# aicodix/modem

Measured on AMD Instinct MI355X. Metric: decoded frames/sec + BER, mode-6 8kHz OFDM, batch 65536, 1/2/4/8 MI355X, higher is better.
Workload: dtype f32

## Files before the change

modem_amd/csrc/dev_common.h:

```cpp
#pragma once
#include <hip/hip_runtime.h>
#include <stdint.h>

#if defined(BACK_WALK) || defined(DEMOD_QA_LDS) || defined(DEMOD_RAW_AHEAD) || defined(DEMOD_SWZ) || defined(DEMOD_TWR_BYTES) || defined(POLAR_NT_LEVEL) || defined(POLAR_WPB) || defined(POLAR_XB1) || defined(POLAR_XB2) || defined(POLAR_XB3) || defined(SYNC_FFT_IN_LDS) || defined(SYNC_PER) || defined(SYNC_SPLIT_8K) || defined(SYNC_SPLIT_ROUNDS) || defined(SYNC_WAVES) || defined(SYNC_WAVES_SPLIT_MONO) || defined(TS_CAP) || defined(TS_MARGIN) || defined(TS_MORE_OCC) || defined(TS_MORE_WAVES_N) || defined(TS_OPEN_MARGIN) || defined(TS_OPEN_NEED) || defined(TS_OWN_ATAN) || defined(TS_ROWS_PER_WG) || defined(TS_UNC_STEPS) || defined(TX_NT_LDS) || defined(TX_TW_GLOBAL)
#error "a frozen tuning macro was passed with -D: edit a patched copy of the source instead (tools/experiments/ts_stage_probe.py shows how)"
#endif

namespace rx {

template <int RATE> struct RateCfg {
	static constexpr int SL = (int)((1280L * RATE) / 8000);
	static constexpr int FILTER_LEN = (((21 * RATE) / 8000) & ~3) | 1;
	static constexpr int GL = SL / 8;
	static constexpr int STRIDE = SL + GL;
	static constexpr int HS = SL / 2;
	static constexpr int BUFFER_LEN = 6 * STRIDE;
	static constexpr int SEARCH_POS = BUFFER_LEN - 4 * STRIDE;
	static constexpr int MATCH_LEN = GL | 1;
	static constexpr int MATCH_DEL = (MATCH_LEN - 1) / 2;
};
inline bool rate_supported(int rate) { return rate == 8000 || rate == 16000 || rate == 44100 || rate == 48000; }
inline int rate_symbol_len(int rate) { return (int)((1280L * rate) / 8000); }
inline int rate_filter_len(int rate) { return (((21 * rate) / 8000) & ~3) | 1; }
#define RX_RATE_SWITCH(rate, ...) \
// ... 27 lines not shown
constexpr int MESG_BITS_MAX = 44096;
constexpr int MESG_BYTES_MAX = 5512;

struct ModeDesc { int cols, rows, mod_bits, cons_bits, mesg_bits, table; };
__host__ __device__ inline ModeDesc mode_desc(int mode)
{
	ModeDesc m;
	m.table = mode >= 10;
	m.cons_bits = m.table ? 64512 : 64800;
	m.mesg_bits = m.table ? 44096 : 43808;
	switch (mode) {
	case 6: m.cols = 432; m.mod_bits = 3; break;
	case 7: m.cols = 400; m.mod_bits = 3; break;
	case 8: m.cols = 400; m.mod_bits = 2; break;
	case 9: m.cols = 360; m.mod_bits = 2; break;
	case 10: m.cols = 512; m.mod_bits = 3; break;
	case 11: m.cols = 384; m.mod_bits = 3; break;
	case 12: m.cols = 384; m.mod_bits = 2; break;
	default: m.cols = 256; m.mod_bits = 2; break;
	}
	m.rows = (m.cons_bits / m.mod_bits) / m.cols;
	return m;
}

struct cf { float re, im; };

__device__ __forceinline__ cf mk(float re, float im) { cf r; r.re = re; r.im = im; return r; }
__device__ __forceinline__ cf cadd(cf a, cf b) { return mk(a.re + b.re, a.im + b.im); }
__device__ __forceinline__ cf csub(cf a, cf b) { return mk(a.re - b.re, a.im - b.im); }
__device__ __forceinline__ cf cmul(cf a, cf b) { return mk(a.re * b.re - a.im * b.im, a.re * b.im + a.im * b.re); }
__device__ __forceinline__ cf cconj(cf a) { return mk(a.re, -a.im); }
__device__ __forceinline__ float cnorm(cf a) { return a.re * a.re + a.im * a.im; }
__device__ __forceinline__ cf cmul_negj(cf a) { return mk(a.im, -a.re); }

__device__ __forceinline__ cf demod_or_erase(cf curr, cf prev)
{
	float d = cnorm(prev);
	if (!(d > 0.f))
		return mk(0.f, 0.f);
	cf n = cmul(curr, cconj(prev));
	cf c = mk(n.re / d, n.im / d);
	if (!(cnorm(c) <= 4.f))
		return mk(0.f, 0.f);
	return c;
}

__device__ __forceinline__ cf psk4_hard_map(cf c)
{
	const float r = 0.70710678118654752440f;
	return mk(r * (c.re < 0.f ? -1.f : 1.f), r * (c.im < 0.f ? -1.f : 1.f));
}
__device__ __forceinline__ cf psk8_hard_map(cf c)
{
	const float cos_pi_8 = 0.92387953251128675613f, sin_pi_8 = 0.38268343236508977173f;
	float b1 = c.re < 0.f ? -1.f : 1.f;
	float b2 = c.im < 0.f ? -1.f : 1.f;
	bool swap = fabsf(c.re) < fabsf(c.im);
	float real = swap ? sin_pi_8 : cos_pi_8, imag = swap ? cos_pi_8 : sin_pi_8;
	return mk(real * b1, imag * b2);
}

__device__ __forceinline__ cf phasor(float omega, long k)
{
	double a = (double)omega * (double)k;
	const double inv2pi = 0.15915494309189533577, twopi = 6.28318530717958647692;
	a -= twopi * rint(a * inv2pi);
	float s, c;
	sincosf((float)a, &s, &c);
	return mk(c, s);
}

__device__ __forceinline__ float div_32767(float x)
{
	const float c = 1.0f / 32767.f;
	const float q0 = x * c;
	return __builtin_fmaf(__builtin_fmaf(-32767.f, q0, x), c, q0);
}
__device__ __forceinline__ float div_127(float x)
{
	const float c = 1.0f / 127.f;
	const float q0 = x * c;
	return __builtin_fmaf(__builtin_fmaf(-127.f, q0, x), c, q0);
}

template <int FMT> __device__ __forceinline__ float2 iq_sample(const void *in, size_t i)
{
	if (FMT == 0) {
		const short2 v = ((const short2 *)in)[i];
		return make_float2(div_32767((float)v.x), div_32767((float)v.y));
	}
	if (FMT == 1) {
		const unsigned v = ((const uint16_t *)in)[i];
		return make_float2(div_127((float)((int)(v & 255u) - 128)), div_127((float)((int)(v >> 8) - 128)));
	}
	return ((const float2 *)in)[i];
}

__device__ __forceinline__ void phase_phasor(unsigned phase, float &cs, float &sn)
{
	const float x = (float)(int)phase * (1.f / 4294967296.f);
	sincospif(2.f * x, &sn, &cs);
}

__device__ __forceinline__ long long floor_div(long long a, int d)
{
	const long long q = a / d;
	return q * d > a ? q - 1 : q;
}

template <int OFMT> __device__ __forceinline__ void iq_store(void *out, long long t0, int t, float wr, float wi)
{
	if (OFMT == 0) {
		const float re = fminf(fmaxf(wr + 0.f, -1.f), 1.f), im = fminf(fmaxf(wi + 0.f, -1.f), 1.f);
		((short2 *)out)[t0 + t] = make_short2((short)nearbyintf(32767.f * re), (short)nearbyintf(32767.f * im));
	} else {
		((float2 *)out)[t0 + t] = make_float2(wr + 0.f, wi + 0.f);
	}
}

template <int V> struct IntC { static constexpr int value = V; };
struct SampleSrc {
	const void *base;
	int fmt;
	int channels;
	long n;
	const cf *analytic;
	__device__ __forceinline__ cf at(long i) const
	{
		if (i < 0 || i >= n)
			return mk(0.f, 0.f);
		if (analytic)
			return analytic[i];
		if (fmt == 0) {
			short2 v = ((const short2 *)base)[i];
			return mk(div_32767((float)v.x), div_32767((float)v.y));
		}
		return pair_other(i);
	}
	__device__ __forceinline__ cf pair_other(long i) const
	{
		if (fmt == 1) {
			const unsigned v = ((const uint16_t *)base)[i];
			return mk(div_127((float)((int)(v & 255u) - 128)), div_127((float)((int)(v >> 8) - 128)));
		}
		const float2 v = ((const float2 *)base)[i];
		return mk(v.x, v.y);
	}
	__device__ __forceinline__ int mode() const { return analytic ? 0 : (fmt == 0 ? 1 : 2); }
	template <int M> __device__ __forceinline__ cf at_m(long i) const
	{
		if (i < 0 || i >= n)
			return mk(0.f, 0.f);
		if (M == 0)
			return analytic[i];
		if (M == 1) {
			short2 v = ((const short2 *)base)[i];
			return mk(div_32767((float)v.x), div_32767((float)v.y));
		}
		return pair_other(i);
	}
	template <class F> __device__ __forceinline__ void with_mode(F f) const
	{
		const int m = mode();
		if (m == 0) f(IntC<0>{});
		else if (m == 1) f(IntC<1>{});
		else f(IntC<2>{});
// ... 95 lines not shown
			Bfly<R>::run(v[q]);
		}
	}
	fft_sync<NT>();
	#pragma unroll
	for (int q = 0; q < NB; ++q) {
		int b = tid + q * NT;
		if (b < T) {
			int k = b % P;
			int j = (b - k) * R + k;
			#pragma unroll
			for (int t = 0; t < R; ++t)
				buf[j + t * P] = v[q][t];
		}
	}
	fft_sync<NT>();
}

template <int N, int REM, int P, int NT, int TWN, int TWC> struct FftPlan {
	static constexpr int R = REM % 5 == 0 ? 5 : REM % 7 == 0 ? 7 : REM % 3 == 0 ? 3 : REM % 4 == 0 ? 4 : 2;
	static constexpr int OWN = P > 1 ? (R - 1) * P : 0;
	using Next = FftPlan<N, REM / R, P * R, NT, TWN, (TWC >= 0 ? TWC + OWN : -1)>;
	static constexpr int COMPACT = OWN + Next::COMPACT;
	static __device__ __forceinline__ void run(cf *buf, const cf *tw, int tid)
	{
		fft_stage<N, R, P, NT, TWN, TWC>(buf, tw, tid);
		Next::run(buf, tw, tid);
	}
	static __device__ __forceinline__ void fill(cf *dst, const cf *src, int tid)
	{
		if (P > 1)
			for (int i = tid; i < OWN; i += NT)
				dst[TWC + i] = src[((i / P + 1) * (i % P)) * (TWN / (P * R))];
		Next::fill(dst, src, tid);
	}
};
template <int N, int P, int NT, int TWN, int TWC> struct FftPlan<N, 1, P, NT, TWN, TWC> {
	static constexpr int COMPACT = 0;
	static __device__ __forceinline__ void run(cf *, const cf *, int) {}
	static __device__ __forceinline__ void fill(cf *, const cf *, int) {}
};
template <int N, int NT, int TWN>
__device__ __forceinline__ void fft_fwd(cf *buf, const cf *tw, int tid)
{
	FftPlan<N, N, 1, NT, TWN, -1>::run(buf, tw, tid);
}
template <int N, int TWN> constexpr int fft_compact_size() { return FftPlan<N, N, 1, 64, TWN, 0>::COMPACT; }
template <int N, int NT, int TWN>
__device__ __forceinline__ void fft_compact_twiddles(cf *dst, const cf *tw, int tid)
{
	FftPlan<N, N, 1, NT, TWN, 0>::fill(dst, tw, tid);
}
template <int N, int NT, int TWN>
__device__ __forceinline__ void fft_fwd_compact(cf *buf, const cf *twc, int tid)
{
	FftPlan<N, N, 1, NT, TWN, 0>::run(buf, twc, tid);
}

__device__ __forceinline__ int swz256(int i) { return i ^ ((i >> 2) & 3) ^ (((i >> 4) & 3) << 2); }
template <int P, int TWC> __device__ __forceinline__ void fft256_stage_swz(cf *buf, const cf *tw, int lane, int sl)
{
	cf v[4];
	const int k = lane % P;
	#pragma unroll
	for (int t = 0; t < 4; ++t) {
		cf x = buf[sl + t * 64];
		if (t && P > 1)
			x = cmul(x, tw[TWC + (t - 1) * P + k]);
		v[t] = x;
	}
	Bfly<4>::run(v);
	fft_sync<64>();
	const int j = (lane - k) * 4 + k;
	#pragma unroll
	for (int t = 0; t < 4; ++t)
		buf[swz256(j + t * P)] = v[t];
	fft_sync<64>();
}

__host__ __device__ constexpr int fft256_pos(int q)
{
	return (q & 192) | ((q & 3) << 4) | (q & 12) | ((q >> 4) & 3);
}
template <int NT> __device__ __forceinline__ void fft256_lane_twiddles(cf *twl, const cf *tw1280, int tid)
{
	for (int i = tid; i < 9 * 64; i += NT) {
		const int l = i & 63, k = (i >> 6) % 3 + 1, step = i / 192;
		const int e = step == 0 ? 5 * (l * k) : step == 1 ? 20 * ((l & 15) * k) : 80 * ((l & 3) * k);
		twl[i] = tw1280[e % 1280];
	}
}
template <int BIT> __device__ __forceinline__ void fft256_xchg(float &A, float &B, int lane)
{
	const int a = __float_as_int(A), b = __float_as_int(B);
	if constexpr (BIT == 5) {
		auto r = __builtin_amdgcn_permlane32_swap((unsigned)a, (unsigned)b, false, false);
		A = __int_as_float((int)r[0]); B = __int_as_float((int)r[1]);
	} else if constexpr (BIT == 4) {
		auto r = __builtin_amdgcn_permlane16_swap((unsigned)a, (unsigned)b, false, false);
		A = __int_as_float((int)r[0]); B = __int_as_float((int)r[1]);
	} else if constexpr (BIT == 3) {
		A = __int_as_float(__builtin_amdgcn_update_dpp(a, b, 0x128, 0xf, 0xC, false));
		B = __int_as_float(__builtin_amdgcn_update_dpp(b, a, 0x128, 0xf, 0x3, false));
	} else if constexpr (BIT == 2) {
		A = __int_as_float(__builtin_amdgcn_update_dpp(a, b, 0x114, 0xf, 0xA, false));
		B = __int_as_float(__builtin_amdgcn_update_dpp(b, a, 0x104, 0xf, 0x5, false));
	} else {
		constexpr int CTRL = BIT == 1 ? 0x4E : 0xB1;
		const int pb = __builtin_amdgcn_update_dpp(0, b, CTRL, 0xf, 0xf, true), pa = __builtin_amdgcn_update_dpp(0, a, CTRL, 0xf, 0xf, true);
		const bool set = (lane >> BIT) & 1;
		A = __int_as_float(set ? pb : a);
		B = __int_as_float(set ? b : pa);
	}
}
template <int HI, int LO> __device__ __forceinline__ void fft256_transpose(cf (&v)[4], int lane)
{
	fft256_xchg<HI>(v[0].re, v[2].re, lane); fft256_xchg<HI>(v[0].im, v[2].im, lane);
	fft256_xchg<HI>(v[1].re, v[3].re, lane); fft256_xchg<HI>(v[1].im, v[3].im, lane);
	fft256_xchg<LO>(v[0].re, v[1].re, lane); fft256_xchg<LO>(v[0].im, v[1].im, lane);
	fft256_xchg<LO>(v[2].re, v[3].re, lane); fft256_xchg<LO>(v[2].im, v[3].im, lane);
}
__device__ __forceinline__ void fft256_regs(cf *buf, const cf *twl, int lane, int sl)
{
	cf v[4];
	#pragma unroll
	for (int t = 0; t < 4; ++t)
		v[t] = buf[sl + t * 64];
	Bfly<4>::run(v);
	#pragma unroll
	for (int k = 1; k < 4; ++k)
		v[k] = cmul(v[k], twl[(k - 1) * 64 + lane]);
	fft256_transpose<5, 4>(v, lane);
	Bfly<4>::run(v);
	#pragma unroll
	for (int k = 1; k < 4; ++k)
		v[k] = cmul(v[k], twl[(3 + k - 1) * 64 + lane]);
	fft256_transpose<3, 2>(v, lane);
	Bfly<4>::run(v);
	#pragma unroll
	for (int k = 1; k < 4; ++k)
		v[k] = cmul(v[k], twl[(6 + k - 1) * 64 + lane]);
	fft256_transpose<1, 0>(v, lane);
	Bfly<4>::run(v);
	fft_sync<64>();
	#pragma unroll
	for (int t = 0; t < 4; ++t)
		buf[lane + t * 64] = v[t];
	fft_sync<64>();
}

__device__ __forceinline__ long uniform_l(long v)
{
	const int lo = __builtin_amdgcn_readfirstlane((int)v), hi = __builtin_amdgcn_readfirstlane((int)(v >> 32));
	return ((long)hi << 32) | (long)(unsigned)lo;
}
__device__ __forceinline__ float uniform_f(float v) { return __int_as_float(__builtin_amdgcn_readfirstlane(__float_as_int(v))); }
__device__ __forceinline__ double shfl_d(double v, int src)
{
	int lo = __double2loint(v), hi = __double2hiint(v);
	lo = __shfl(lo, src);
	hi = __shfl(hi, src);
	return __hiloint2double(hi, lo);
}
__device__ __forceinline__ double shfl_up_d(double v, int d)
{
	int lo = __double2loint(v), hi = __double2hiint(v);
	lo = __shfl_up(lo, d);
	hi = __shfl_up(hi, d);
	return __hiloint2double(hi, lo);
}
__device__ __forceinline__ double shfl_xor_d(double v, int m)
{
	int lo = __double2loint(v), hi = __double2hiint(v);
	lo = __shfl_xor(lo, m);
	hi = __shfl_xor(hi, m);
	return __hiloint2double(hi, lo);
}
template <int CTRL, int ROW_MASK = 0xf> __device__ __forceinline__ float dpp_f(float v)
{
	return __int_as_float(__builtin_amdgcn_update_dpp(0, __float_as_int(v), CTRL, ROW_MASK, 0xf, false));
}
template <int CTRL, int ROW_MASK = 0xf> __device__ __forceinline__ double dpp_d(double v)
{
	const int lo = __builtin_amdgcn_update_dpp(0, __double2loint(v), CTRL, ROW_MASK, 0xf, false);
	const int hi = __builtin_amdgcn_update_dpp(0, __double2hiint(v), CTRL, ROW_MASK, 0xf, false);
	return __hiloint2double(hi, lo);
}
template <class T> struct WScan;
template <> struct WScan<float> {
	static __device__ __forceinline__ float run(float v, const float (&w)[6], float w16, float w32)
	{
		v = fmaf(w[0], dpp_f<0x111>(v), v);
		v = fmaf(w[1], dpp_f<0x112>(v), v);
		v = fmaf(w[2], dpp_f<0x114>(v), v);
		v = fmaf(w[3], dpp_f<0x118>(v), v);
		v = fmaf(w16, dpp_f<0x142, 0xa>(v), v);
		v = fmaf(w32, dpp_f<0x143, 0xc>(v), v);
		return v;
	}
};
template <> struct WScan<double> {
	static __device__ __forceinline__ double run(double v, const double (&w)[7], double w16, double w32)
	{
		v = fma(w[0], dpp_d<0x111>(v), v);
		v = fma(w[1], dpp_d<0x112>(v), v);
		v = fma(w[2], dpp_d<0x114>(v), v);
		v = fma(w[3], dpp_d<0x118>(v), v);
		v = fma(w16, dpp_d<0x142, 0xa>(v), v);
		v = fma(w32, dpp_d<0x143, 0xc>(v), v);
		return v;
	}
};
__device__ __forceinline__ double wave_scan_incl(double v, int lane)
{
	#pragma unroll
	for (int d = 1; d < 64; d <<= 1) {
		double o = shfl_up_d(v, d);
		if (lane >= d)
			v += o;
	}
	return v;
}
__device__ __forceinline__ double wave_sum_d(double v)
{
	#pragma unroll
	for (int m = 32; m; m >>= 1)
// ... 152 lines not shown
```

modem_amd/csrc/k_demod.hip:

```cpp
#include "dev_common.h"
#include "kernels.h"
#include "mono_front.h"

namespace rx {

#define DEMOD_CONS_OUT(R) ((R) != 44100)
template <int RATE> struct DifCfg {
	static constexpr int SL = RateCfg<RATE>::SL;
#define DEMOD_DIF_W(R) ((R) == 48000 ? 3 : (R) == 44100 ? 2 : 1)
	static constexpr int W = DEMOD_DIF_W(RATE);
	static constexpr int R1 = SL % 5 == 0 ? 5 : 7, NS = SL / R1, NT = 64 * W * R1;
	static constexpr int NQ = (NS + NT - 1) / NT;
#define DEMOD_TWR_BYTES 8192
#ifndef DEMOD_WAVES_8K
#define DEMOD_WAVES_8K 7
#endif
#define DEMOD_DIF_WAVES(R) ((R) >= 44100 ? 3 : (R) == 8000 ? DEMOD_WAVES_8K : 5)
#ifndef DEMOD_TWR_8K
#define DEMOD_TWR_8K 1
#endif
	static constexpr bool TWR_LDS = ((R1 - 1) * NS * 8 <= DEMOD_TWR_BYTES && (RATE != 8000 || DEMOD_TWR_8K)) || SL == 7056;
	static constexpr int WAVES = DEMOD_DIF_WAVES(RATE);
};

#define DEMOD_PREFETCH_NQ(R) ((R) >= 44100 ? 2 : 1)
#define DEMOD_SWZ 1
#ifndef DEMOD_REGS
#define DEMOD_REGS 1
#endif

#ifndef DEMOD_MONO_WAVES
#define DEMOD_MONO_WAVES 5
#endif
template <int RATE, int MONO, class FB = FrameBatch>
__global__ __launch_bounds__(DifCfg<RATE>::NT, MONO == 2 ? DEMOD_MONO_WAVES : DifCfg<RATE>::WAVES) void k_demod(FB fb, cf *__restrict__ z_all, MonoArgs ma, Tables tb,
	const SyncState *__restrict__ st_all, cf *__restrict__ cons_all, cf *__restrict__ carr_all)
{
	constexpr int SYMBOL_LEN = RateCfg<RATE>::SL, SYM_STRIDE = RateCfg<RATE>::STRIDE, GUARD_LEN = RateCfg<RATE>::GL;
	const int f = blockIdx.x, tid = threadIdx.x, wave = tid >> 6, lane = tid & 63;
	const SyncState st = st_all[f];
	if (!st.okay)
		return;
	const int fs = batch_source(fb, f);
	SampleSrc src{ batch_base(fb, fs), fb.fmt, fb.channels, batch_len(fb, fs),
		fb.channels == 1 ? z_all + (size_t)f * fb.samples_per_frame : nullptr };
	const ModeDesc md = mode_desc(st.oper_mode);
	cf *cons = cons_all + (size_t)f * CONS_MAX;
	const long body0 = st.sc_start + 2 * SYM_STRIDE;
	const float omega = -st.cfo_rad;
	const int code_off = -md.cols / 2;
	{
		typedef DifCfg<RATE> DC;
		constexpr int NT = DC::NT, R1 = DC::R1, NS = DC::NS, NQ = DC::NQ;
		static_assert(R1 * NS == SYMBOL_LEN, "plan");
		constexpr int TWC = fft_compact_size<NS, SYMBOL_LEN>();
		__shared__ cf row[R1 * NS];
		constexpr bool REGS = DEMOD_REGS && DEMOD_SWZ && NS == 256 && DC::W == 1;
		__shared__ cf tw_sub[REGS ? 1 : TWC];
		__shared__ cf twl[REGS ? 9 * 64 : 1];
		__shared__ cf tw_r[DC::TWR_LDS ? (R1 - 1) * NS : 1];
		__shared__ cf rotA[R1], rotQ[NQ], symrot[ROWS_MAX + 1];
		constexpr int PC_E = NT >= COLS_MAX ? 1 : 2, PC_T = NT >= COLS_MAX ? COLS_MAX : NT;
		__shared__ cf prevc[PC_E][DEMOD_CONS_OUT(RATE) ? PC_T : 1];
		constexpr int MPER = 5, MTH = SYM_STRIDE / MPER, YOFF = (GUARD_LEN - 32) / MPER * MPER, YB = GUARD_LEN - YOFF;
		static_assert(MONO != 2 || (MTH * MPER == SYM_STRIDE && MTH <= NT && NS == 256 && NQ == 1 && MonoCfg<RATE>::REACH <= 32 && GUARD_LEN % MPER == 0
			&& (MTH + 63) / 64 == 5 && MTH % 64 == 32), "span layout");
		__shared__ float ybuf[MONO == 2 ? SYM_STRIDE - YOFF : 1];
		__shared__ float mwe[5];
		if constexpr (REGS)
			fft256_lane_twiddles<NT>(twl, tb.tw_sym, tid);
		else
			fft_compact_twiddles<NS, NT, SYMBOL_LEN>(tw_sub, tb.tw_sym, tid);
		if (DC::TWR_LDS)
			for (int i = tid; i < (R1 - 1) * NS; i += NT)
				tw_r[i] = tb.tw_sym[(i / NS + 1) * (i % NS)];
		if (tid < R1)
			rotA[tid] = phasor(omega, (long)NS * tid);
		if (tid >= 64 && tid < 64 + NQ)
			rotQ[tid - 64] = phasor(omega, (long)NT * (tid - 64));
		if (tid <= md.rows)
			symrot[tid] = phasor(omega, (long)tid * SYM_STRIDE);
		const cf p0 = phasor(omega, (long)SYMBOL_LEN + tid);
		__syncthreads();
#define DEMOD_QA_LDS 0
		constexpr bool QA_LDS = MONO == 2 || DEMOD_QA_LDS;
		cf qa[NQ == 1 ? R1 : 1];
		if (NQ == 1) {
			#pragma unroll
			for (int a = 0; a < R1; ++a)
				qa[a] = (a && !QA_LDS) ? cmul(p0, rotA[a]) : p0;
		}
		int coff[2];
		#pragma unroll
		for (int e = 0; e < 2; ++e) {
			const int i = tid + NT * e, k = (i + code_off + SYMBOL_LEN) % SYMBOL_LEN;
			coff[e] = i < md.cols ? (k % R1) * NS + (REGS ? fft256_pos(k / R1) : (DEMOD_SWZ && NS == 256 && DC::W == 1) ? swz256(k / R1) : k / R1) : -1;
		}
		const MonoFrame mfr = mono_frame(fb, ma.ck, ma.ck_per_frame, f);
		const long span0 = MONO == 2 ? uniform_l(body0 - GUARD_LEN) : 0;
		float mS = 0.f, mAspan = 1.f, mAw = 1.f, mAwave = 1.f;
		const float mg = ma.g * mfr.scale(), mb = ma.b * mfr.scale();
		float mAlane = 1.f, mW16 = 1.f, mW32 = 1.f, my0[MPER] = {};
		int mxi[MPER] = {};
		bool mpacked = false;
		const bool mfloat = mfr.fmt == 2;
		auto mono_raw = [&](int sym) {
			const long e0 = span0 + (long)sym * SYM_STRIDE;
			const int n32 = (int)mfr.n;
			if (tid < MTH) {
				mpacked = mfr.fmt == 0 && e0 >= 0 && e0 + SYM_STRIDE <= mfr.n;
				if (mpacked) {
					typedef uint32_t __attribute__((aligned(2))) word_at_2;
					const int16_t *q = (const int16_t *)mfr.base + e0 + tid * MPER;
					mxi[0] = (int)((const word_at_2 *)q)[0];
					mxi[1] = (int)((const word_at_2 *)q)[1];
					mxi[2] = (int)((const uint16_t *)q)[4];
				} else {
					#pragma unroll
					for (int i = 0; i < MPER; ++i) {
						const int j = (int)e0 + tid * MPER + i, jc = min(max(j, 0), n32 - 1);
						int v;
						if (mfr.fmt == 0) v = ((const int16_t *)mfr.base)[jc];
						else if (mfr.fmt == 1) v = (int)((const uint8_t *)mfr.base)[jc] - 128;
						else v = ((const int *)mfr.base)[jc];
						mxi[i] = j == jc ? v : 0;
					}
				}
			}
		};
		auto mono_part1 = [&]() {
			float acc = 0.f, sl[MPER], mx[MPER];
			if (mpacked) {
				mx[0] = (float)(short)(mxi[0] & 0xffff); mx[1] = (float)(mxi[0] >> 16);
				mx[2] = (float)(short)(mxi[1] & 0xffff); mx[3] = (float)(mxi[1] >> 16);
				mx[4] = (float)(short)mxi[2];
			} else {
				#pragma unroll
				for (int i = 0; i < MPER; ++i)
					mx[i] = mfloat ? __int_as_float(mxi[i]) : (float)mxi[i];
			}
			#pragma unroll
			for (int i = 0; i < MPER; ++i) {
				sl[i] = acc;
				acc = fmaf(ma.a, acc, mg * mx[i]);
			}
			const float v = WScan<float>::run(acc, ma.astep5, mW16, mW32);
			if (lane == (wave < 4 ? 63 : 31))
				mwe[wave] = v;
			const float cw0 = dpp_f<0x138>(v);
			my0[0] = fmaf(mb, mx[0], -cw0);
			#pragma unroll
			for (int i = 1; i < MPER; ++i)
				my0[i] = fmaf(mb, mx[i], -fmaf(ma.apw[i - 1], cw0, sl[i]));
		};
		auto mono_part2 = [&]() {
			float st = 0.f, stw = 0.f;
			#pragma unroll
			for (int w = 0; w < 4; ++w) {
				st = fmaf(mAwave, st, mwe[w]);
				if (w < wave)
					stw = st;
			}
			const float cl = mAlane * uniform_f(fmaf(mAw, mS, stw));
			mS = uniform_f(fmaf(mAspan, mS, fmaf(ma.astep5[5], st, mwe[4])));
			if (tid >= YOFF / MPER && tid < MTH) {
				float *yo = ybuf + (tid * MPER - YOFF);
				yo[0] = my0[0] - cl;
				#pragma unroll
				for (int i = 1; i < MPER; ++i)
					yo[i] = fmaf(-ma.apw[i - 1], cl, my0[i]);
			}
		};
		if constexpr (MONO == 2) {
			mAlane = (float)mono_pow((double)ma.a, MPER * lane);
			mW16 = (float)mono_pow((double)ma.a, MPER * ((lane & 15) + 1));
			mW32 = (float)mono_pow((double)ma.a, MPER * ((lane & 31) + 1));
			mAspan = uniform_f((float)mono_pow((double)ma.a, SYM_STRIDE));
			mAw = uniform_f((float)mono_pow((double)ma.a, 64 * MPER * wave));
			mAwave = (float)ma.awave5;
			if (span0 > 0) {
				const long c0 = span0 / MONO_CK * MONO_CK;
				const int gap = (int)(span0 - c0);
				const double term = lane < gap ? (double)mg * (double)mfr.raw(c0 + lane) * mono_pow((double)ma.a, gap - 1 - lane) : 0.0;
				mS = uniform_f((float)(mono_pow((double)ma.a, gap) * mfr.state_before(c0) + wave_sum_d(term)));
			}
			mono_raw(0);
			mono_part1();
			__syncthreads();
			mono_part2();
			mono_raw(1);
			__syncthreads();
		}
		constexpr bool TWR_REG = !DC::TWR_LDS && NQ * (R1 - 1) <= 8 && RATE != 8000;
		cf twq[TWR_REG ? NQ : 1][TWR_REG ? R1 - 1 : 1];
		if constexpr (TWR_REG) {
			#pragma unroll
			for (int q = 0; q < NQ; ++q)
				#pragma unroll
				for (int r = 1; r < R1; ++r)
					twq[q][r - 1] = tid + NT * q < NS ? tb.tw_sym[r * (tid + NT * q)] : mk(0.f, 0.f);
		}
		constexpr bool QA_REG2 = NQ == 2 && R1 == 5 && RATE == 48000;
		cf qa2[QA_REG2 ? NQ : 1][QA_REG2 ? R1 : 1];
		if constexpr (QA_REG2) {
			#pragma unroll
			for (int q = 0; q < NQ; ++q) {
				const cf pq = q ? cmul(p0, rotQ[q]) : p0;
				#pragma unroll
				for (int a = 0; a < R1; ++a)
					qa2[q][a] = a ? cmul(pq, rotA[a]) : pq;
			}
		}
		auto symbols = [&](auto M) {
		constexpr int MODE = decltype(M)::value;
		cf pre[NQ][R1];
#define DEMOD_RAW_AHEAD 1
		constexpr bool RAW = DEMOD_RAW_AHEAD && MODE == 1 && MONO == 0 && NQ <= DEMOD_PREFETCH_NQ(RATE);
		int praw[RAW ? NQ : 1][RAW ? R1 : 1];
		auto fetch = [&](int sym) {
			const long t0 = body0 + (long)sym * SYM_STRIDE;
			if constexpr (MONO == 2) {
				const bool inside = t0 >= 0 && t0 + SYMBOL_LEN <= src.n;
				if (tid < NS) {
					#pragma unroll
					for (int a = 0; a < R1; ++a) {
						const int m = tid + NS * a;
						cf zv = mono_hilbert<RATE>(ma.co, [&](int k) { return ybuf[YB + m - MonoCfg<RATE>::REACH + k]; });
						if (!inside && (t0 + m < 0 || t0 + m >= src.n))
							zv = mk(0.f, 0.f);
						pre[0][a] = zv;
						__builtin_amdgcn_sched_barrier(0);
					}
				}
				return;
			}
			if (MODE == 1 && sym <= md.rows && t0 >= 0 && t0 + SYMBOL_LEN <= src.n) {
				const short2 *p = (const short2 *)src.base + t0;
				#pragma unroll
				for (int q = 0; q < NQ; ++q) {
					const int np = tid + NT * q;
					if (np < NS) {
						#pragma unroll
						for (int a = 0; a < R1; ++a) {
							if constexpr (RAW)
								praw[q][a] = ((const int *)p)[np + NS * a];
							else {
								const short2 x = p[np + NS * a];
								pre[q][a] = mk(div_32767((float)x.x), div_32767((float)x.y));
							}
						}
					}
				}
			} else if constexpr (RAW) {
				#pragma unroll
				for (int q = 0; q < NQ; ++q) {
					const int np = tid + NT * q;
					#pragma unroll
					for (int a = 0; a < R1; ++a) {
						const long i = t0 + np + NS * a;
						praw[q][a] = (np < NS && sym <= md.rows && i >= 0 && i < src.n) ? ((const int *)src.base)[i] : 0;
					}
				}
			} else {
				#pragma unroll
				for (int q = 0; q < NQ; ++q) {
					const int np = tid + NT * q;
					#pragma unroll
					for (int a = 0; a < R1; ++a)
						pre[q][a] = (np < NS && sym <= md.rows) ? src.template at_m<MODE>(t0 + np + NS * a) : mk(0.f, 0.f);
				}
			}
		};
		constexpr bool AHEAD = NQ <= DEMOD_PREFETCH_NQ(RATE) && MONO == 0;
		if (AHEAD)
			fetch(0);
		cf *carr = carr_all + (size_t)f * CARR_MAX;
		for (int s = 0; s <= md.rows; ++s) {
			if (!AHEAD)
				fetch(s);
			#pragma unroll
			for (int q = 0; q < NQ; ++q) {
				const int np = tid + NT * q;
				if (np < NS) {
					cf v[R1];
					if constexpr (RAW) {
						#pragma unroll
						for (int a = 0; a < R1; ++a)
							pre[q][a] = mk(div_32767((float)(short)(praw[q][a] & 0xffff)), div_32767((float)(praw[q][a] >> 16)));
					}
					if (NQ == 1) {
						#pragma unroll
						for (int a = 0; a < R1; ++a)
							v[a] = cmul(pre[q][a], (QA_LDS && a) ? cmul(p0, rotA[a]) : qa[a]);
					} else if constexpr (QA_REG2) {
						#pragma unroll
						for (int a = 0; a < R1; ++a)
							v[a] = cmul(pre[q][a], qa2[q][a]);
					} else {
						const cf pq = q ? cmul(p0, rotQ[q]) : p0;
						#pragma unroll
						for (int a = 0; a < R1; ++a)
							v[a] = cmul(pre[q][a], a ? cmul(pq, rotA[a]) : pq);
					}
					Bfly<R1>::run(v);
					const int npw = (DEMOD_SWZ && NS == 256 && DC::W == 1) ? swz256(np) : np;
					row[npw] = v[0];
					#pragma unroll
					for (int r = 1; r < R1; ++r)
						row[r * NS + npw] = cmul(v[r], DC::TWR_LDS ? tw_r[(r - 1) * NS + np] : TWR_REG ? twq[TWR_REG ? q : 0][TWR_REG ? r - 1 : 0] : tb.tw_sym[r * np]);
				}
			}
			if (AHEAD)
				fetch(s + 1);
			__syncthreads();
			if constexpr (REGS) {
				fft256_regs(row + wave * NS, twl, lane, swz256(lane));
			} else if constexpr (DEMOD_SWZ && NS == 256 && DC::W == 1) {
				cf *sub = row + wave * NS;
				const int sl = swz256(lane);
				fft256_stage_swz<1, 0>(sub, tw_sub, lane, sl);
				fft256_stage_swz<4, 0>(sub, tw_sub, lane, sl);
				fft256_stage_swz<16, 12>(sub, tw_sub, lane, sl);
				fft256_stage_swz<64, 60>(sub, tw_sub, lane, sl);
			} else
				fft_fwd_compact<NS, 64 * DC::W, SYMBOL_LEN>(row + (tid / (64 * DC::W)) * NS, tw_sub, tid % (64 * DC::W));
			if constexpr (MONO == 2)
				if (s < md.rows)
					mono_part1();
			__syncthreads();
			const cf w = symrot[s];
			#pragma unroll
			for (int e = 0; e < 2; ++e)
				if (coff[e] >= 0) {
					const cf cur = cmul(row[coff[e]], w);
					if constexpr (DEMOD_CONS_OUT(RATE)) {
						if (s > 0)
							cons[(size_t)(s - 1) * md.cols + tid + NT * e] = demod_or_erase(cur, prevc[e][tid]);
						prevc[e][tid] = cur;
					} else
						carr[tid + NT * e] = cur;
				}
			carr += md.cols;
			if constexpr (MONO == 2)
				if (s < md.rows) {
					mono_part2();
					if (s + 2 <= md.rows)
						mono_raw(s + 2);
				}
			__syncthreads();
		}
		};
		if constexpr (MONO != 0)
			symbols(IntC<0>{});
		else
			src.with_mode(symbols);
	}
}

template <int RATE>
__global__ __launch_bounds__(256) void k_fft_debug(int len, int sign, const cf *__restrict__ in, cf *__restrict__ out, const cf *__restrict__ tw)
{
	constexpr int SYMBOL_LEN = RateCfg<RATE>::SL;
	const int f = blockIdx.x, tid = threadIdx.x;
	__shared__ cf buf[SYMBOL_LEN];
	for (int i = tid; i < len; i += 256) {
		cf v = in[(size_t)f * len + i];
		buf[i] = sign > 0 ? cconj(v) : v;
	}
	__syncthreads();
	if (len == SYMBOL_LEN) fft_fwd<SYMBOL_LEN, 256, SYMBOL_LEN>(buf, tw, tid);
	else fft_fwd<SYMBOL_LEN / 2, 256, SYMBOL_LEN>(buf, tw, tid);
	for (int i = tid; i < len; i += 256)
		out[(size_t)f * len + i] = sign > 0 ? cconj(buf[i]) : buf[i];
}

bool demod_forms_cons(int rate) { return DEMOD_CONS_OUT(rate); }
void launch_demod_sources(hipStream_t s, int rate, int n, SourceBatch fb, Tables tb, const SyncState *st, cf *cons, cf *carr)
{
	RX_RATE_SWITCH(rate, hipLaunchKernelGGL((k_demod<RATE, 0, SourceBatch>), dim3(n), dim3(DifCfg<RATE>::NT), 0, s, fb, nullptr, MonoArgs{}, tb, st, cons, carr));
}
void launch_demod_bank(hipStream_t s, int rate, int n, WindowBatch fb, Tables tb, const SyncState *st, cf *cons, cf *carr)
{
	RX_RATE_SWITCH(rate, hipLaunchKernelGGL((k_demod<RATE, 0, WindowBatch>), dim3(n), dim3(DifCfg<RATE>::NT), 0, s, fb, nullptr, MonoArgs{}, tb, st, cons, carr));
}
void launch_demod(hipStream_t s, int rate, int n, FrameBatch fb, cf *z, const MonoArgs &ma, Tables tb, const SyncState *st, cf *cons, cf *carr)
{
	if (fb.channels == 1 && mono_fused(rate)) {
		hipLaunchKernelGGL((k_demod<8000, 2>), dim3(n), dim3(DifCfg<8000>::NT), 0, s, fb, z, ma, tb, st, cons, carr);
	} else {
		RX_RATE_SWITCH(rate, hipLaunchKernelGGL((k_demod<RATE, 0>), dim3(n), dim3(DifCfg<RATE>::NT), 0, s, fb, z, ma, tb, st, cons, carr));
	}
}
void launch_fft_debug(hipStream_t s, int rate, int n, int len, int sign, const cf *in, cf *out, Tables tb)
{
	RX_RATE_SWITCH(rate, hipLaunchKernelGGL(k_fft_debug<RATE>, dim3(n), dim3(256), 0, s, len, sign, in, out, tb.tw_sym));
}

}
```

Before: 1.876 million.

## Use packed-f32 VOP3P complex arithmetic in the 8 kHz demodulator

```diff
diff --git a/modem_amd/csrc/dev_common.h b/modem_amd/csrc/dev_common.h
--- a/modem_amd/csrc/dev_common.h
+++ b/modem_amd/csrc/dev_common.h
@@ -133,6 +133,110 @@
 	const float q0 = x * c;
 	return __builtin_fmaf(__builtin_fmaf(-127.f, q0, x), c, q0);
 }
+
+typedef float pf __attribute__((ext_vector_type(2)));
+#define RX_PK2(op, d, a, b, mods) asm(op " %0, %1, %2 " mods : "=v"(d) : "v"(a), "v"(b))
+#define RX_PK3(op, d, a, b, c, mods) asm(op " %0, %1, %2, %3 " mods : "=v"(d) : "v"(a), "v"(b), "v"(c))
+#define RX_PK2S(op, d, k, b, mods) asm(op " %0, %1, %2 " mods : "=v"(d) : "s"(k), "v"(b))
+#define RX_PK3S(op, d, k, b, c, mods) asm(op " %0, %1, %2, %3 " mods : "=v"(d) : "s"(k), "v"(b), "v"(c))
+struct CxLegacy {
+	typedef cf T;
+	static __device__ __forceinline__ T make(float re, float im) { return mk(re, im); }
+	static __device__ __forceinline__ T from(cf a) { return a; }
+	static __device__ __forceinline__ cf to(T a) { return a; }
+	template <int ORD = 0> static __device__ __forceinline__ T mul(T a, T b) { return cmul(a, b); }
+	static __device__ __forceinline__ T mul_conj(T a, T b) { return cmul(a, cconj(b)); }
+	static __device__ __forceinline__ T from_s16x2(int raw) { return mk(div_32767((float)(short)(raw & 0xffff)), div_32767((float)(raw >> 16))); }
+};
+struct CxScalar {
+	typedef cf T;
+	typedef float K2[2];
+	static __device__ __forceinline__ T make(float re, float im) { return mk(re, im); }
+	static __device__ __forceinline__ T from(cf a) { return a; }
+	static __device__ __forceinline__ cf to(T a) { return a; }
+	static __device__ __forceinline__ T add(T a, T b) { return mk(a.re + b.re, a.im + b.im); }
+	static __device__ __forceinline__ T sub(T a, T b) { return mk(a.re - b.re, a.im - b.im); }
+	static __device__ __forceinline__ T conj(T a) { return mk(a.re, -a.im); }
+	static __device__ __forceinline__ T mul_negj(T a) { return mk(a.im, -a.re); }
+	static __device__ __forceinline__ T mul_j(T a) { return mk(-a.im, a.re); }
+	static __device__ __forceinline__ T add_negj(T a, T b) { return mk(a.re + b.im, a.im - b.re); }
+	static __device__ __forceinline__ T sub_negj(T a, T b) { return mk(a.re - b.im, a.im + b.re); }
+	template <int ORD = 0> static __device__ __forceinline__ T mul(T a, T b)
+	{
+		return mk(__builtin_fmaf(a.re, b.re, -(a.im * b.im)), ORD ? __builtin_fmaf(a.re, b.im, a.im * b.re) : __builtin_fmaf(a.im, b.re, a.re * b.im));
+	}
+	static __device__ __forceinline__ float norm(T a) { return __builtin_fmaf(a.re, a.re, a.im * a.im); }
+	static __device__ __forceinline__ T mul_conj(T a, T b)
+	{
+		return mk(__builtin_fmaf(a.re, b.re, a.im * b.im), __builtin_fmaf(a.im, b.re, -(a.re * b.im)));
+	}
+	template <int H> static __device__ __forceinline__ T scale(const K2 &k, T a) { return mk(k[H] * a.re, k[H] * a.im); }
+	template <int H> static __device__ __forceinline__ T fma(const K2 &k, T a, T c) { return mk(__builtin_fmaf(k[H], a.re, c.re), __builtin_fmaf(k[H], a.im, c.im)); }
+	template <int H> static __device__ __forceinline__ T fms(const K2 &k, T a, T c) { return mk(__builtin_fmaf(k[H], a.re, -c.re), __builtin_fmaf(k[H], a.im, -c.im)); }
+	static __device__ __forceinline__ T from_s16x2(int raw) { return mk(div_32767((float)(short)(raw & 0xffff)), div_32767((float)(raw >> 16))); }
+};
+struct CxPacked {
+	typedef pf T;
+	typedef pf K2;
+	static __device__ __forceinline__ T make(float re, float im) { T r; r.x = re; r.y = im; return r; }
+	static __device__ __forceinline__ T from(cf a) { return make(a.re, a.im); }
+	static __device__ __forceinline__ cf to(T a) { return mk(a.x, a.y); }
+	static __device__ __forceinline__ T add(T a, T b) { T d; RX_PK2("v_pk_add_f32", d, a, b, ""); return d; }
+	static __device__ __forceinline__ T sub(T a, T b) { T d; RX_PK2("v_pk_add_f32", d, a, b, "neg_lo:[0,1] neg_hi:[0,1]"); return d; }
+	static __device__ __forceinline__ T conj(T a) { T d; RX_PK2("v_pk_mul_f32", d, a, make(1.f, 1.f), "neg_hi:[1,0]"); return d; }
+	static __device__ __forceinline__ T add_negj(T a, T b) { T d; RX_PK2("v_pk_add_f32", d, a, b, "op_sel:[0,1] op_sel_hi:[1,0] neg_hi:[0,1]"); return d; }
+	static __device__ __forceinline__ T sub_negj(T a, T b) { T d; RX_PK2("v_pk_add_f32", d, a, b, "op_sel:[0,1] op_sel_hi:[1,0] neg_lo:[0,1]"); return d; }
+	static __device__ __forceinline__ T mul_negj(T a) { return add_negj(make(0.f, 0.f), a); }
+	static __device__ __forceinline__ T mul_j(T a) { return sub_negj(make(0.f, 0.f), a); }
+	template <int ORD = 0> static __device__ __forceinline__ T mul(T a, T b)
+	{
+		T t, d;
+		if (ORD) {
+			RX_PK2("v_pk_mul_f32", t, a, b, "op_sel:[1,1] op_sel_hi:[1,0]");
+			RX_PK3("v_pk_fma_f32", d, a, b, t, "op_sel:[0,0,0] op_sel_hi:[0,1,1] neg_lo:[0,0,1]");
+		} else {
+			RX_PK2("v_pk_mul_f32", t, a, b, "op_sel:[1,1] op_sel_hi:[0,1]");
+			RX_PK3("v_pk_fma_f32", d, a, b, t, "op_sel:[0,0,0] op_sel_hi:[1,0,1] neg_lo:[0,0,1]");
+		}
+		return d;
+	}
+	static __device__ __forceinline__ float norm(T a) { return __builtin_fmaf(a.x, a.x, a.y * a.y); }
+	static __device__ __forceinline__ T mul_conj(T a, T b)
+	{
+		T t, d;
+		RX_PK2("v_pk_mul_f32", t, a, b, "op_sel:[1,1] op_sel_hi:[0,1]");
+		RX_PK3("v_pk_fma_f32", d, a, b, t, "op_sel:[0,0,0] op_sel_hi:[1,0,1] neg_hi:[0,0,1]");
+		return d;
+	}
+	template <int H> static __device__ __forceinline__ T scale(const K2 &k, T a)
+	{
+		T d;
+		if (H) RX_PK2S("v_pk_mul_f32", d, k, a, "op_sel:[1,0] op_sel_hi:[1,1]"); else RX_PK2S("v_pk_mul_f32", d, k, a, "op_sel:[0,0] op_sel_hi:[0,1]");
+		return d;
+	}
+	template <int H> static __device__ __forceinline__ T fma(const K2 &k, T a, T c)
+	{
+		T d;
+		if (H) RX_PK3S("v_pk_fma_f32", d, k, a, c, "op_sel:[1,0,0] op_sel_hi:[1,1,1]"); else RX_PK3S("v_pk_fma_f32", d, k, a, c, "op_sel:[0,0,0] op_sel_hi:[0,1,1]");
+		return d;
+	}
+	template <int H> static __device__ __forceinline__ T fms(const K2 &k, T a, T c)
+	{
+		T d;
+		if (H) RX_PK3S("v_pk_fma_f32", d, k, a, c, "op_sel:[1,0,0] op_sel_hi:[1,1,1] neg_lo:[0,0,1] neg_hi:[0,0,1]");
+		else RX_PK3S("v_pk_fma_f32", d, k, a, c, "op_sel:[0,0,0] op_sel_hi:[0,1,1] neg_lo:[0,0,1] neg_hi:[0,0,1]");
+		return d;
+	}
+	static __device__ __forceinline__ T from_s16x2(int raw)
+	{
+		const K2 k = { 1.0f / 32767.f, -32767.f };
+		const T x = make((float)(short)(raw & 0xffff), (float)(raw >> 16));
+		const T q0 = scale<0>(k, x), r = fma<1>(k, q0, x);
+		T d;
+		RX_PK3S("v_pk_fma_f32", d, k, r, q0, "op_sel:[0,0,0] op_sel_hi:[0,1,1]");
+		return d;
+	}
+};
 
 template <int FMT> __device__ __forceinline__ float2 iq_sample(const void *in, size_t i)
 {
@@ -394,12 +498,12 @@
 {
 	return (q & 192) | ((q & 3) << 4) | (q & 12) | ((q >> 4) & 3);
 }
-template <int NT> __device__ __forceinline__ void fft256_lane_twiddles(cf *twl, const cf *tw1280, int tid)
+template <int NT, class A = CxLegacy> __device__ __forceinline__ void fft256_lane_twiddles(typename A::T *twl, const cf *tw1280, int tid)
 {
 	for (int i = tid; i < 9 * 64; i += NT) {
 		const int l = i & 63, k = (i >> 6) % 3 + 1, step = i / 192;
 		const int e = step == 0 ? 5 * (l * k) : step == 1 ? 20 * ((l & 15) * k) : 80 * ((l & 3) * k);
-		twl[i] = tw1280[e % 1280];
+		twl[i] = A::from(tw1280[e % 1280]);
 	}
 }
 template <int BIT> __device__ __forceinline__ void fft256_xchg(float &A, float &B, int lane)
@@ -425,35 +529,64 @@
 		B = __int_as_float(set ? b : pa);
 	}
 }
-template <int HI, int LO> __device__ __forceinline__ void fft256_transpose(cf (&v)[4], int lane)
-{
-	fft256_xchg<HI>(v[0].re, v[2].re, lane); fft256_xchg<HI>(v[0].im, v[2].im, lane);
-	fft256_xchg<HI>(v[1].re, v[3].re, lane); fft256_xchg<HI>(v[1].im, v[3].im, lane);
-	fft256_xchg<LO>(v[0].re, v[1].re, lane); fft256_xchg<LO>(v[0].im, v[1].im, lane);
-	fft256_xchg<LO>(v[2].re, v[3].re, lane); fft256_xchg<LO>(v[2].im, v[3].im, lane);
-}
-__device__ __forceinline__ void fft256_regs(cf *buf, const cf *twl, int lane, int sl)
-{
-	cf v[4];
+template <int BIT, class A> __device__ __forceinline__ void fft256_xchg_c(typename A::T &a, typename A::T &b, int lane)
+{
+	const cf ca = A::to(a), cb = A::to(b);
+	float ar = ca.re, ai = ca.im, br = cb.re, bi = cb.im;
+	fft256_xchg<BIT>(ar, br, lane); fft256_xchg<BIT>(ai, bi, lane);
+	a = A::make(ar, ai); b = A::make(br, bi);
+}
+template <int HI, int LO, class A> __device__ __forceinline__ void fft256_transpose(typename A::T (&v)[4], int lane)
+{
+	fft256_xchg_c<HI, A>(v[0], v[2], lane); fft256_xchg_c<HI, A>(v[1], v[3], lane);
+	fft256_xchg_c<LO, A>(v[0], v[1], lane); fft256_xchg_c<LO, A>(v[2], v[3], lane);
+}
+template <class A> __device__ __forceinline__ void bfly4(typename A::T *v)
+{
+	typedef typename A::T T;
+	const T s0 = A::add(v[0], v[2]), s1 = A::sub(v[0], v[2]);
+	const T s2 = A::add(v[1], v[3]), d = A::sub(v[1], v[3]);
+	v[0] = A::add(s0, s2); v[1] = A::add_negj(s1, d); v[2] = A::sub(s0, s2); v[3] = A::sub_negj(s1, d);
+}
+template <class A> __device__ __forceinline__ void bfly5(typename A::T *v)
+{
+	typedef typename A::T T;
+	const typename A::K2 kc = { 0.30901699437494742410f, -0.80901699437494742410f }, ks = { 0.95105651629515357212f, 0.58778525229247312917f };
+	const T a1 = A::add(v[1], v[4]), a2 = A::add(v[2], v[3]);
+	const T b1 = A::sub(v[1], v[4]), b2 = A::sub(v[2], v[3]);
+	const T m1 = A::template fma<1>(kc, a2, A::template fma<0>(kc, a1, v[0]));
+	const T m2 = A::template fma<0>(kc, a2, A::template fma<1>(kc, a1, v[0]));
+	const T n1 = A::template fma<1>(ks, b2, A::template scale<0>(ks, b1));
+	const T n2 = A::template fms<1>(ks, b1, A::template scale<0>(ks, b2));
+	v[0] = A::add(A::add(a1, a2), v[0]);
+	v[1] = A::add_negj(m1, n1); v[4] = A::sub_negj(m1, n1);
+	v[2] = A::add_negj(m2, n2); v[3] = A::sub_negj(m2, n2);
+}
+template <class A = CxLegacy, int ORD = 0> __device__ __forceinline__ void fft256_regs(typename A::T *buf, const typename A::T *twl, int lane, int sl)
+{
+	typedef typename A::T T;
+	constexpr bool LEGACY = __is_same(A, CxLegacy);
+	auto bfly = [](T *v) { if constexpr (LEGACY) Bfly<4>::run(v); else bfly4<A>(v); };
+	T v[4];
 	#pragma unroll
 	for (int t = 0; t < 4; ++t)
 		v[t] = buf[sl + t * 64];
-	Bfly<4>::run(v);
+	bfly(v);
 	#pragma unroll
 	for (int k = 1; k < 4; ++k)
-		v[k] = cmul(v[k], twl[(k - 1) * 64 + lane]);
-	fft256_transpose<5, 4>(v, lane);
-	Bfly<4>::run(v);
+		v[k] = A::template mul<(ORD >> 0) & 1>(v[k], twl[(k - 1) * 64 + lane]);
+	fft256_transpose<5, 4, A>(v, lane);
+	bfly(v);
 	#pragma unroll
 	for (int k = 1; k < 4; ++k)
-		v[k] = cmul(v[k], twl[(3 + k - 1) * 64 + lane]);
-	fft256_transpose<3, 2>(v, lane);
-	Bfly<4>::run(v);
+		v[k] = A::template mul<(ORD >> 1) & 1>(v[k], twl[(3 + k - 1) * 64 + lane]);
+	fft256_transpose<3, 2, A>(v, lane);
+	bfly(v);
 	#pragma unroll
 	for (int k = 1; k < 4; ++k)
-		v[k] = cmul(v[k], twl[(6 + k - 1) * 64 + lane]);
-	fft256_transpose<1, 0>(v, lane);
-	Bfly<4>::run(v);
+		v[k] = A::template mul<(ORD >> 2) & 1>(v[k], twl[(6 + k - 1) * 64 + lane]);
+	fft256_transpose<1, 0, A>(v, lane);
+	bfly(v);
 	fft_sync<64>();
 	#pragma unroll
 	for (int t = 0; t < 4; ++t)
diff --git a/modem_amd/csrc/k_demod.hip b/modem_amd/csrc/k_demod.hip
--- a/modem_amd/csrc/k_demod.hip
+++ b/modem_amd/csrc/k_demod.hip
@@ -1,6 +1,7 @@
 #include "dev_common.h"
 #include "kernels.h"
 #include "mono_front.h"
+#include <cstdlib>
 
 namespace rx {
 
@@ -32,11 +33,43 @@
 #ifndef DEMOD_MONO_WAVES
 #define DEMOD_MONO_WAVES 5
 #endif
-template <int RATE, int MONO, class FB = FrameBatch>
+#ifndef DEMOD_MUL_ORD
+#define DEMOD_MUL_ORD 64
+#endif
+#define MORD(b) ((DEMOD_MUL_ORD >> (b)) & 1)
+#ifndef DEMOD_PK_PHASES
+#define DEMOD_PK_PHASES 7
+#endif
+template <int RATE, bool PACKED> struct DemodArith { typedef CxLegacy A; };
+template <> struct DemodArith<8000, false> { typedef CxScalar A; };
+template <> struct DemodArith<8000, true> { typedef CxPacked A; };
+template <class A> __device__ __forceinline__ cf demod_or_erase_a(typename A::T curr, typename A::T prev)
+{
+	if constexpr (__is_same(A, CxLegacy))
+		return demod_or_erase(curr, prev);
+	else {
+		const float d = A::norm(prev);
+		if (!(d > 0.f))
+			return mk(0.f, 0.f);
+		const cf n = A::to(A::mul_conj(curr, prev));
+		const cf c = mk(n.re / d, n.im / d);
+		if (!(CxScalar::norm(c) <= 4.f))
+			return mk(0.f, 0.f);
+		return c;
+	}
+}
+template <int RATE, int MONO, class FB = FrameBatch, bool PACKED = false>
 __global__ __launch_bounds__(DifCfg<RATE>::NT, MONO == 2 ? DEMOD_MONO_WAVES : DifCfg<RATE>::WAVES) void k_demod(FB fb, cf *__restrict__ z_all, MonoArgs ma, Tables tb,
 	const SyncState *__restrict__ st_all, cf *__restrict__ cons_all, cf *__restrict__ carr_all)
 {
 	constexpr int SYMBOL_LEN = RateCfg<RATE>::SL, SYM_STRIDE = RateCfg<RATE>::STRIDE, GUARD_LEN = RateCfg<RATE>::GL;
+	static_assert(!PACKED || RATE == 8000, "the packed arithmetic is the 8 kHz demodulator's");
+	typedef typename DemodArith<RATE, PACKED && (DEMOD_PK_PHASES & 1)>::A A;
+	typedef typename DemodArith<RATE, PACKED && (DEMOD_PK_PHASES & 2)>::A AT;
+	typedef typename DemodArith<RATE, PACKED && (DEMOD_PK_PHASES & 4)>::A AC;
+	typedef typename A::T ct;
+	typedef typename AT::T ctt;
+	typedef typename AC::T ctc;
 	const int f = blockIdx.x, tid = threadIdx.x, wave = tid >> 6, lane = tid & 63;
 	const SyncState st = st_all[f];
 	if (!st.okay)
@@ -54,41 +87,43 @@
 		constexpr int NT = DC::NT, R1 = DC::R1, NS = DC::NS, NQ = DC::NQ;
 		static_assert(R1 * NS == SYMBOL_LEN, "plan");
 		constexpr int TWC = fft_compact_size<NS, SYMBOL_LEN>();
-		__shared__ cf row[R1 * NS];
+		__shared__ __attribute__((aligned(16))) cf row_lds[R1 * NS];
+		ct *const row = (ct *)row_lds;
 		constexpr bool REGS = DEMOD_REGS && DEMOD_SWZ && NS == 256 && DC::W == 1;
 		__shared__ cf tw_sub[REGS ? 1 : TWC];
-		__shared__ cf twl[REGS ? 9 * 64 : 1];
-		__shared__ cf tw_r[DC::TWR_LDS ? (R1 - 1) * NS : 1];
-		__shared__ cf rotA[R1], rotQ[NQ], symrot[ROWS_MAX + 1];
+		__shared__ ctt twl[REGS ? 9 * 64 : 1];
+		__shared__ ct tw_r[DC::TWR_LDS ? (R1 - 1) * NS : 1];
+		__shared__ ct rotA[R1], rotQ[NQ];
+		__shared__ ctc symrot[ROWS_MAX + 1];
 		constexpr int PC_E = NT >= COLS_MAX ? 1 : 2, PC_T = NT >= COLS_MAX ? COLS_MAX : NT;
-		__shared__ cf prevc[PC_E][DEMOD_CONS_OUT(RATE) ? PC_T : 1];
+		__shared__ ctc prevc[PC_E][DEMOD_CONS_OUT(RATE) ? PC_T : 1];
 		constexpr int MPER = 5, MTH = SYM_STRIDE / MPER, YOFF = (GUARD_LEN - 32) / MPER * MPER, YB = GUARD_LEN - YOFF;
 		static_assert(MONO != 2 || (MTH * MPER == SYM_STRIDE && MTH <= NT && NS == 256 && NQ == 1 && MonoCfg<RATE>::REACH <= 32 && GUARD_LEN % MPER == 0
 			&& (MTH + 63) / 64 == 5 && MTH % 64 == 32), "span layout");
 		__shared__ float ybuf[MONO == 2 ? SYM_STRIDE - YOFF : 1];
 		__shared__ float mwe[5];
 		if constexpr (REGS)
-			fft256_lane_twiddles<NT>(twl, tb.tw_sym, tid);
+			fft256_lane_twiddles<NT, AT>(twl, tb.tw_sym, tid);
 		else
 			fft_compact_twiddles<NS, NT, SYMBOL_LEN>(tw_sub, tb.tw_sym, tid);
 		if (DC::TWR_LDS)
 			for (int i = tid; i < (R1 - 1) * NS; i += NT)
-				tw_r[i] = tb.tw_sym[(i / NS + 1) * (i % NS)];
+				tw_r[i] = A::from(tb.tw_sym[(i / NS + 1) * (i % NS)]);
 		if (tid < R1)
-			rotA[tid] = phasor(omega, (long)NS * tid);
+			rotA[tid] = A::from(phasor(omega, (long)NS * tid));
 		if (tid >= 64 && tid < 64 + NQ)
-			rotQ[tid - 64] = phasor(omega, (long)NT * (tid - 64));
+			rotQ[tid - 64] = A::from(phasor(omega, (long)NT * (tid - 64)));
 		if (tid <= md.rows)
-			symrot[tid] = phasor(omega, (long)tid * SYM_STRIDE);
-		const cf p0 = phasor(omega, (long)SYMBOL_LEN + tid);
+			symrot[tid] = AC::from(phasor(omega, (long)tid * SYM_STRIDE));
+		const ct p0 = A::from(phasor(omega, (long)SYMBOL_LEN + tid));
 		__syncthreads();
 #define DEMOD_QA_LDS 0
 		constexpr bool QA_LDS = MONO == 2 || DEMOD_QA_LDS;
-		cf qa[NQ == 1 ? R1 : 1];
+		ct qa[NQ == 1 ? R1 : 1];
 		if (NQ == 1) {
 			#pragma unroll
 			for (int a = 0; a < R1; ++a)
-				qa[a] = (a && !QA_LDS) ? cmul(p0, rotA[a]) : p0;
+				qa[a] = (a && !QA_LDS) ? A::template mul<MORD(0)>(p0, rotA[a]) : p0;
 		}
 		int coff[2];
 		#pragma unroll
@@ -192,28 +227,28 @@
 			__syncthreads();
 		}
 		constexpr bool TWR_REG = !DC::TWR_LDS && NQ * (R1 - 1) <= 8 && RATE != 8000;
-		cf twq[TWR_REG ? NQ : 1][TWR_REG ? R1 - 1 : 1];
+		ct twq[TWR_REG ? NQ : 1][TWR_REG ? R1 - 1 : 1];
 		if constexpr (TWR_REG) {
 			#pragma unroll
 			for (int q = 0; q < NQ; ++q)
 				#pragma unroll
 				for (int r = 1; r < R1; ++r)
-					twq[q][r - 1] = tid + NT * q < NS ? tb.tw_sym[r * (tid + NT * q)] : mk(0.f, 0.f);
+					twq[q][r - 1] = A::from(tid + NT * q < NS ? tb.tw_sym[r * (tid + NT * q)] : mk(0.f, 0.f));
 		}
 		constexpr bool QA_REG2 = NQ == 2 && R1 == 5 && RATE == 48000;
-		cf qa2[QA_REG2 ? NQ : 1][QA_REG2 ? R1 : 1];
+		ct qa2[QA_REG2 ? NQ : 1][QA_REG2 ? R1 : 1];
 		if constexpr (QA_REG2) {
 			#pragma unroll
 			for (int q = 0; q < NQ; ++q) {
-				const cf pq = q ? cmul(p0, rotQ[q]) : p0;
+				const ct pq = q ? A::mul(p0, rotQ[q]) : p0;
 				#pragma unroll
 				for (int a = 0; a < R1; ++a)
-					qa2[q][a] = a ? cmul(pq, rotA[a]) : pq;
+					qa2[q][a] = a ? A::mul(pq, rotA[a]) : pq;
 			}
 		}
 		auto symbols = [&](auto M) {
 		constexpr int MODE = decltype(M)::value;
-		cf pre[NQ][R1];
+		ct pre[NQ][R1];
 #define DEMOD_RAW_AHEAD 1
 		constexpr bool RAW = DEMOD_RAW_AHEAD && MODE == 1 && MONO == 0 && NQ <= DEMOD_PREFETCH_NQ(RATE);
 		int praw[RAW ? NQ : 1][RAW ? R1 : 1];
@@ -228,7 +263,7 @@
 						cf zv = mono_hilbert<RATE>(ma.co, [&](int k) { return ybuf[YB + m - MonoCfg<RATE>::REACH + k]; });
 						if (!inside && (t0 + m < 0 || t0 + m >= src.n))
 							zv = mk(0.f, 0.f);
-						pre[0][a] = zv;
+						pre[0][a] = A::from(zv);
 						__builtin_amdgcn_sched_barrier(0);
 					}
 				}
@@ -246,7 +281,7 @@
 								praw[q][a] = ((const int *)p)[np + NS * a];
 							else {
 								const short2 x = p[np + NS * a];
-								pre[q][a] = mk(div_32767((float)x.x), div_32767((float)x.y));
+								pre[q][a] = A::from(mk(div_32767((float)x.x), div_32767((float)x.y)));
 							}
 						}
 					}
@@ -267,7 +302,7 @@
 					const int np = tid + NT * q;
 					#pragma unroll
 					for (int a = 0; a < R1; ++a)
-						pre[q][a] = (np < NS && sym <= md.rows) ? src.template at_m<MODE>(t0 + np + NS * a) : mk(0.f, 0.f);
+						pre[q][a] = A::from((np < NS && sym <= md.rows) ? src.template at_m<MODE>(t0 + np + NS * a) : mk(0.f, 0.f));
 				}
 			}
 		};
@@ -282,63 +317,67 @@
 			for (int q = 0; q < NQ; ++q) {
 				const int np = tid + NT * q;
 				if (np < NS) {
-					cf v[R1];
+					ct v[R1];
 					if constexpr (RAW) {
 						#pragma unroll
 						for (int a = 0; a < R1; ++a)
-							pre[q][a] = mk(div_32767((float)(short)(praw[q][a] & 0xffff)), div_32767((float)(praw[q][a] >> 16)));
+							pre[q][a] = A::from_s16x2(praw[q][a]);
 					}
 					if (NQ == 1) {
+						v[0] = A::template mul<(MONO == 2 ? 1 : MORD(1))>(pre[q][0], qa[0]);
 						#pragma unroll
-						for (int a = 0; a < R1; ++a)
-							v[a] = cmul(pre[q][a], (QA_LDS && a) ? cmul(p0, rotA[a]) : qa[a]);
+						for (int a = 1; a < R1; ++a)
+							v[a] = A::template mul<MORD(1)>(pre[q][a], QA_LDS ? A::template mul<MORD(0)>(p0, rotA[a]) : qa[a]);
 					} else if constexpr (QA_REG2) {
 						#pragma unroll
 						for (int a = 0; a < R1; ++a)
-							v[a] = cmul(pre[q][a], qa2[q][a]);
+							v[a] = A::mul(pre[q][a], qa2[q][a]);
 					} else {
-						const cf pq = q ? cmul(p0, rotQ[q]) : p0;
+						const ct pq = q ? A::mul(p0, rotQ[q]) : p0;
 						#pragma unroll
 						for (int a = 0; a < R1; ++a)
-							v[a] = cmul(pre[q][a], a ? cmul(pq, rotA[a]) : pq);
-					}
-					Bfly<R1>::run(v);
+							v[a] = A::mul(pre[q][a], a ? A::mul(pq, rotA[a]) : pq);
+					}
+					if constexpr (RATE == 8000)
+						bfly5<A>(v);
+					else
+						Bfly<R1>::run(v);
 					const int npw = (DEMOD_SWZ && NS == 256 && DC::W == 1) ? swz256(np) : np;
 					row[npw] = v[0];
 					#pragma unroll
 					for (int r = 1; r < R1; ++r)
-						row[r * NS + npw] = cmul(v[r], DC::TWR_LDS ? tw_r[(r - 1) * NS + np] : TWR_REG ? twq[TWR_REG ? q : 0][TWR_REG ? r - 1 : 0] : tb.tw_sym[r * np]);
+						row[r * NS + npw] = A::template mul<MORD(2)>(v[r], DC::TWR_LDS ? tw_r[(r - 1) * NS + np] : TWR_REG ? twq[TWR_REG ? q : 0][TWR_REG ? r - 1 : 0] : A::from(tb.tw_sym[r * np]));
 				}
 			}
 			if (AHEAD)
 				fetch(s + 1);
 			__syncthreads();
 			if constexpr (REGS) {
-				fft256_regs(row + wave * NS, twl, lane, swz256(lane));
+				fft256_regs<AT, (DEMOD_MUL_ORD >> 3) & 7>((ctt *)row_lds + wave * NS, twl, lane, swz256(lane));
 			} else if constexpr (DEMOD_SWZ && NS == 256 && DC::W == 1) {
-				cf *sub = row + wave * NS;
+				cf *sub = row_lds + wave * NS;
 				const int sl = swz256(lane);
 				fft256_stage_swz<1, 0>(sub, tw_sub, lane, sl);
 				fft256_stage_swz<4, 0>(sub, tw_sub, lane, sl);
 				fft256_stage_swz<16, 12>(sub, tw_sub, lane, sl);
 				fft256_stage_swz<64, 60>(sub, tw_sub, lane, sl);
 			} else
-				fft_fwd_compact<NS, 64 * DC::W, SYMBOL_LEN>(row + (tid / (64 * DC::W)) * NS, tw_sub, tid % (64 * DC::W));
+				fft_fwd_compact<NS, 64 * DC::W, SYMBOL_LEN>(row_lds + (tid / (64 * DC::W)) * NS, tw_sub, tid % (64 * DC::W));
 			if constexpr (MONO == 2)
 				if (s < md.rows)
 					mono_part1();
 			__syncthreads();
-			const cf w = symrot[s];
+			const ctc w = symrot[s];
 			#pragma unroll
 			for (int e = 0; e < 2; ++e)
 				if (coff[e] >= 0) {
-					const cf cur = cmul(row[coff[e]], w);
+					const ctc cur = AC::template mul<MORD(6)>(((const ctc *)row_lds)[coff[e]], w);
 					if constexpr (DEMOD_CONS_OUT(RATE)) {
 						if (s > 0)
-							cons[(size_t)(s - 1) * md.cols + tid + NT * e] = demod_or_erase(cur, prevc[e][tid]);
+							cons[(size_t)(s - 1) * md.cols + tid + NT * e] = demod_or_erase_a<AC>(cur, prevc[e][tid]);
 						prevc[e][tid] = cur;
 					} else
-						carr[tid + NT * e] = cur;
+						carr[tid + NT * e] = AC::to(cur);
 				}
 			carr += md.cols;
 			if constexpr (MONO == 2)
@@ -375,20 +414,33 @@
 }
 
 bool demod_forms_cons(int rate) { return DEMOD_CONS_OUT(rate); }
+static bool demod_scalar()
+{
+	const char *e = std::getenv("OFDMRX_DEMOD_SCALAR");
+	return e && e[0] && e[0] != '0';
+}
+template <int RATE, int MONO, class FB>
+static void demod_launch(hipStream_t s, int n, FB fb, cf *z, const MonoArgs &ma, Tables tb, const SyncState *st, cf *cons, cf *carr)
+{
+	if (RATE == 8000 && !demod_scalar())
+		hipLaunchKernelGGL((k_demod<RATE, MONO, FB, RATE == 8000>), dim3(n), dim3(DifCfg<RATE>::NT), 0, s, fb, z, ma, tb, st, cons, carr);
+	else
+		hipLaunchKernelGGL((k_demod<RATE, MONO, FB, false>), dim3(n), dim3(DifCfg<RATE>::NT), 0, s, fb, z, ma, tb, st, cons, carr);
+}
 void launch_demod_sources(hipStream_t s, int rate, int n, SourceBatch fb, Tables tb, const SyncState *st, cf *cons, cf *carr)
 {
-	RX_RATE_SWITCH(rate, hipLaunchKernelGGL((k_demod<RATE, 0, SourceBatch>), dim3(n), dim3(DifCfg<RATE>::NT), 0, s, fb, nullptr, MonoArgs{}, tb, st, cons, carr));
+	RX_RATE_SWITCH(rate, demod_launch<RATE, 0, SourceBatch>(s, n, fb, nullptr, MonoArgs{}, tb, st, cons, carr));
 }
 void launch_demod_bank(hipStream_t s, int rate, int n, WindowBatch fb, Tables tb, const SyncState *st, cf *cons, cf *carr)
 {
-	RX_RATE_SWITCH(rate, hipLaunchKernelGGL((k_demod<RATE, 0, WindowBatch>), dim3(n), dim3(DifCfg<RATE>::NT), 0, s, fb, nullptr, MonoArgs{}, tb, st, cons, carr));
+	RX_RATE_SWITCH(rate, demod_launch<RATE, 0, WindowBatch>(s, n, fb, nullptr, MonoArgs{}, tb, st, cons, carr));
 }
 void launch_demod(hipStream_t s, int rate, int n, FrameBatch fb, cf *z, const MonoArgs &ma, Tables tb, const SyncState *st, cf *cons, cf *carr)
 {
 	if (fb.channels == 1 && mono_fused(rate)) {
-		hipLaunchKernelGGL((k_demod<8000, 2>), dim3(n), dim3(DifCfg<8000>::NT), 0, s, fb, z, ma, tb, st, cons, carr);
+		demod_launch<8000, 2, FrameBatch>(s, n, fb, z, ma, tb, st, cons, carr);
 	} else {
-		RX_RATE_SWITCH(rate, hipLaunchKernelGGL((k_demod<RATE, 0>), dim3(n), dim3(DifCfg<RATE>::NT), 0, s, fb, z, ma, tb, st, cons, carr));
+		RX_RATE_SWITCH(rate, demod_launch<RATE, 0, FrameBatch>(s, n, fb, z, ma, tb, st, cons, carr));
 	}
 }
 void launch_fft_debug(hipStream_t s, int rate, int n, int len, int sign, const cf *in, cf *out, Tables tb)
```

Result: no change. 1.878 million (median of 4 runs) (+0.1%).
